# jgsimard/big-dreamer

Measured on AMD Instinct MI355X. Metric: latent transitions/sec (RSSM + imagination) at batch=50 chunk=50 H=15, higher is better.
Workload: dtype f32

## Files before the change

### big_dreamer_amd/csrc/bd_device.h

```cpp
#pragma once
#include <hip/hip_runtime.h>
#include <stdint.h>

namespace bd {

typedef float floatx4 __attribute__((ext_vector_type(4)));

#ifndef BD_WAVES
#define BD_WAVES 4
#endif
constexpr int kWaves = BD_WAVES;
constexpr int kThreads = kWaves * 64;
constexpr int kFragFloats = 256;

__device__ __forceinline__ floatx4 mfma16(float a, float b, floatx4 c) {
    return __builtin_amdgcn_mfma_f32_16x16x4f32(a, b, c, 0, 0, 0);
}

__host__ __device__ __forceinline__ int cdiv(int a, int b) { return (a + b - 1) / b; }

__device__ __forceinline__ int bd_tid() {
    int t = threadIdx.x;
    asm volatile("" : "+v"(t));
    return t;
}
static_assert((kWaves & (kWaves - 1)) == 0, "kWaves must be a power of two");
__device__ __forceinline__ int bd_wave(int tid) { return ((tid >> 6) + (int)blockIdx.x) & (kWaves - 1); }

#define BD_KARGS(T, name) const __attribute__((address_space(4))) T* name = \
    (const __attribute__((address_space(4))) T*)__builtin_amdgcn_kernarg_segment_ptr()
#define BD_KARGS_FRESH(name) asm volatile("" : "+s"(name))

__device__ __forceinline__ void lds_barrier() {
    asm volatile("s_waitcnt lgkmcnt(0)" ::: "memory");
    __builtin_amdgcn_s_barrier();
    asm volatile("" ::: "memory");
}

__device__ __forceinline__ int frag_idx(int row, int k) {
    return ((k >> 4) * 64 + ((k >> 2) & 3) * 16 + row) * 4 + (k & 3);
}

#ifdef BD_EXACT_MATH
__device__ __forceinline__ float elu(float x) { return x > 0.f ? x : expm1f(x); }
__device__ __forceinline__ float sigmoidf(float x) { return 1.f / (1.f + expf(-x)); }
__device__ __forceinline__ float tanh_act(float x) { return tanhf(x); }
__device__ __forceinline__ float softplusf(float x) { return x > 20.f ? x : log1pf(expf(x)); }
__device__ __forceinline__ float one_minus_exp_neg(float x) { return -expm1f(-x); }
#else
__device__ __forceinline__ float elu(float x) { return x > 0.f ? x : __expf(x) - 1.f; }
__device__ __forceinline__ float sigmoidf(float x) { return __builtin_amdgcn_rcpf(1.f + __expf(-x)); }
__device__ __forceinline__ float tanh_act(float x) { return 1.f - 2.f * __builtin_amdgcn_rcpf(__expf(2.f * x) + 1.f); }
__device__ __forceinline__ float softplusf(float x) { return x > 20.f ? x : __logf(1.f + __expf(x)); }
__device__ __forceinline__ float one_minus_exp_neg(float x) { return 1.f - __expf(-x); }
#endif
__device__ __forceinline__ float elu_grad_from_out(float y) { return y > 0.f ? 1.f : y + 1.f; }
__device__ __forceinline__ float act_apply(int act, float x) { return act ? elu(x) : x; }

__device__ __forceinline__ float wave_sum(float v) {
#pragma unroll
    for (int off = 32; off > 0; off >>= 1) v += __shfl_down(v, off, 64);
    return v;
}
__device__ __forceinline__ double wave_sum_d(double v) {
#pragma unroll
    for (int off = 32; off > 0; off >>= 1) v += __shfl_down(v, off, 64);
    return v;
}
__device__ __forceinline__ double block_sum_d(double v, double* red) {
    v = wave_sum_d(v);
    const int lane = threadIdx.x & 63, wave = threadIdx.x >> 6;
    __syncthreads();
    if (lane == 0) red[wave] = v;
    __syncthreads();
    double s = 0.0;
    if (bd_tid() == 0) {
        const int nw = (blockDim.x + 63) >> 6;
        for (int w = 0; w < nw; ++w) s += red[w];
    }
    return s;
}

template <int RT>
__device__ __forceinline__ void load_tile_concat(float* __restrict__ X, int Kb, int row0, int M,
                                                 const float* __restrict__ in0, int ld0, int w0,
                                                 const float* __restrict__ in1, int ld1, int w1,
                                                 float scale = 1.f) {
    const int Kp = Kb * 16;
    for (int idx = bd_tid(); idx < RT * 16 * Kp; idx += blockDim.x) {
        const int r = idx / Kp, k = idx - r * Kp;
        const int grow = row0 + r;
        float v = 0.f;
        if (grow < M) {
            if (k < w0) v = in0[(size_t)grow * ld0 + k];
            else if (k < w0 + w1) v = in1[(size_t)grow * ld1 + (k - w0)];
        }
        X[(r >> 4) * Kb * kFragFloats + frag_idx(r & 15, k)] = v * scale;
    }
}

__host__ __device__ __forceinline__ bool tile_pairs_ok(const float* in0, int ld0, int w0, const float* in1, int ld1) {
    return ((w0 | ld0) & 1) == 0 && ((uintptr_t)in0 & 7) == 0 && (in1 == nullptr || ((ld1 & 1) == 0 && ((uintptr_t)in1 & 7) == 0));
}
template <int RT>
__device__ __forceinline__ void load_tile_concat_pairs(float* __restrict__ X, int Kb, int row0, int M,
                                                       const float* __restrict__ in0, int ld0, int w0,
                                                       const float* __restrict__ in1, int ld1, int w1) {
    typedef float floatx2 __attribute__((ext_vector_type(2)));
    const int tid = bd_tid(), wave = tid >> 6, lane = tid & 63;
    const int Kp = Kb * 16, W = w0 + w1;
    constexpr int kRows = 16 * RT / kWaves;
    constexpr int kBatch = 6;
    static_assert(16 * RT % kWaves == 0, "rows must divide over the waves");
    for (int k = 2 * lane; k < Kp; k += 128) {
#pragma unroll
        for (int b0 = 0; b0 < kRows; b0 += kBatch) {
            floatx2 v[kBatch];
#pragma unroll
            for (int b = 0; b < kBatch; ++b) {
                const int r = wave + (b0 + b) * kWaves, grow = row0 + r;
                v[b] = floatx2{0.f, 0.f};
                if (b0 + b < kRows && grow < M) {
                    if (k < w0) v[b] = *reinterpret_cast<const floatx2*>(in0 + (size_t)grow * ld0 + k);
                    else if (k + 1 < W) v[b] = *reinterpret_cast<const floatx2*>(in1 + (size_t)grow * ld1 + (k - w0));
                    else if (k < W) v[b][0] = in1[(size_t)grow * ld1 + (k - w0)];
                }
            }
#pragma unroll
            for (int b = 0; b < kBatch; ++b) {
                const int r = wave + (b0 + b) * kWaves;
                if (b0 + b < kRows)
                    *reinterpret_cast<floatx2*>(X + (r >> 4) * Kb * kFragFloats + frag_idx(r & 15, k)) = v[b];
            }
        }
    }
}

template <int D, class LoadF, class MmaF>
__device__ __forceinline__ void pipelined_k(int Kb, LoadF&& load, MmaF&& mma) {
    using Frag = decltype(load(0));
    const int G = Kb / D, nt = Kb - G * D;
    Frag A[D], B[D];
    Frag T[D > 1 ? D - 1 : 1];
#pragma unroll
    for (int i = 0; i < D - 1; ++i)
        if (i < nt) T[i] = load(G * D + i);
    if (G > 0) {
#pragma unroll
        for (int i = 0; i < D; ++i) A[i] = load(i);
        int g = 1;
        for (; g + 1 < G; g += 2) {
#pragma unroll
            for (int i = 0; i < D; ++i) B[i] = load(g * D + i);
            __builtin_amdgcn_sched_barrier(0);
#pragma unroll
            for (int i = 0; i < D; ++i) mma(A[i]);
#pragma unroll
            for (int i = 0; i < D; ++i) A[i] = load((g + 1) * D + i);
            __builtin_amdgcn_sched_barrier(0);
#pragma unroll
            for (int i = 0; i < D; ++i) mma(B[i]);
        }
        if (g < G) {
#pragma unroll
            for (int i = 0; i < D; ++i) B[i] = load(g * D + i);
            __builtin_amdgcn_sched_barrier(0);
#pragma unroll
            for (int i = 0; i < D; ++i) mma(A[i]);
#pragma unroll
            for (int i = 0; i < D; ++i) mma(B[i]);
        } else {
#pragma unroll
// ... 486 lines not shown
            const size_t off = (size_t)nb * Kb * 64 + lane;
            const floatx4* __restrict__ W0 = reinterpret_cast<const floatx4*>(seg[s].W0) + off;
            const floatx4* __restrict__ W1 = reinterpret_cast<const floatx4*>(seg[s].W1) + off;
            if (seg[s].W0 != nullptr && seg[s].W1 != nullptr) {
                pipelined_k<2>(
                    Kb, [&](int kb) { return DualFrag{X4[kb * 64], W0[kb * 64], W1[kb * 64]}; },
                    [&](const DualFrag& f) {
#pragma unroll
                        for (int j = 0; j < 4; ++j) {
                            acc0 = mfma16(f.a[j], f.p[j], acc0);
                            acc1 = mfma16(f.a[j], f.q[j], acc1);
                        }
                    });
            } else if (seg[s].W0 != nullptr) {
                for (int kb = 0; kb < Kb; ++kb) {
                    const floatx4 a4 = X4[kb * 64], p4 = W0[kb * 64];
#pragma unroll
                    for (int j = 0; j < 4; ++j) acc0 = mfma16(a4[j], p4[j], acc0);
                }
            } else if (seg[s].W1 != nullptr) {
                for (int kb = 0; kb < Kb; ++kb) {
                    const floatx4 a4 = X4[kb * 64], q4 = W1[kb * 64];
#pragma unroll
                    for (int j = 0; j < 4; ++j) acc1 = mfma16(a4[j], q4[j], acc1);
                }
            }
        }
        epi(nb, acc0, acc1, pf);
    }
}

struct NoPre1 {
    __device__ __forceinline__ NoPreVal operator()(int) const { return NoPreVal{}; }
};
template <int NSEG, class Epi>
__device__ __forceinline__ void tile_linear_dual(const Seg2 (&seg)[NSEG], const float* __restrict__ bias0,
                                                 const float* __restrict__ bias1, int N, Epi&& epi,
                                                 float* __restrict__ scratch = nullptr) {
    tile_linear_dual_pre<NSEG>(seg, bias0, bias1, N, NoPre1{},
                               [&](int nb, floatx4 a0, floatx4 a1, NoPreVal) { epi(nb, a0, a1); }, scratch);
}

template <int NSEG, class PreE, class EpiE>
__device__ __forceinline__ void tile_dual_head_elem(const Seg2 (&seg)[NSEG], const float* __restrict__ bias0,
                                                    const float* __restrict__ bias1, int N, float* __restrict__ scratch,
                                                    PreE&& pre_elem, EpiE&& epi_elem, int sb = -1) {
    const int lane = bd_tid() & 63;
    const int Nb = (N + 15) >> 4, Np = Nb * 16;
    float* __restrict__ plain = scratch + kSplitPartialFloats;
    const int e0 = bd_tid();
    const int row0e = e0 / N, col0e = e0 - row0e * N;
    decltype(pre_elem(0, 0)) pv{};
    BD_DSTAMP(sb, 0);
#ifdef BD_STAMPS
    if (sb >= 0) asm volatile("s_waitcnt vmcnt(0)" ::: "memory");
    BD_DSTAMP(sb, 6);
#endif
    if (e0 < 16 * N) pv = pre_elem(row0e, col0e);
#ifdef BD_STAMPS
    if (sb >= 0) asm volatile("s_waitcnt vmcnt(0)" ::: "memory");
    BD_DSTAMP(sb, 7);
#endif
    BD_DSTAMP(sb, 1);
    tile_linear_dual_pre<NSEG>(
        seg, bias0, bias1, N, NoPre1{},
        [&](int nb, floatx4 a0, floatx4 a1, NoPreVal) {
#pragma unroll
            for (int r = 0; r < 4; ++r) {
                const int o = (4 * (lane >> 4) + r) * Np + nb * 16 + (lane & 15);
                plain[o] = a0[r];
                plain[16 * Np + o] = a1[r];
            }
        },
        Nb <= kSplitPairs ? scratch : nullptr, sb >= 0 ? sb + 16 : -1);
    BD_DSTAMP(sb, 2);
    lds_barrier();
    BD_DSTAMP(sb, 3);
#ifdef BD_STAMPS
    if (sb >= 0) asm volatile("s_waitcnt vmcnt(0)" ::: "memory");
    BD_DSTAMP(sb, 4);
#endif
    if (e0 < 16 * N) epi_elem(row0e, col0e, plain[row0e * Np + col0e], plain[16 * Np + row0e * Np + col0e], pv);
    BD_DSTAMP(sb, 5);
    for (int e = e0 + blockDim.x; e < 16 * N; e += blockDim.x) {
        const int row = e / N, col = e - row * N;
        epi_elem(row, col, plain[row * Np + col], plain[16 * Np + row * Np + col], pre_elem(row, col));
    }
}

#ifndef BD_GRU_PIPE3
#define BD_GRU_PIPE3 0
#endif
#if BD_GRU_PIPE3
#define BD_GRU_PIPE pipelined_k3
#else
#define BD_GRU_PIPE pipelined_k<1>
#endif

struct GruW {
    const float *w_ir, *w_iz, *w_in, *w_hr, *w_hz, *w_hn;
    const float *b_ih, *b_hh;
};

struct GruFrag {
    floatx4 ax, ah, bir, biz, bin, bhr, bhz, bhn;
};

struct GruHalfFrag {
    floatx4 ax, ah, b0, b1;
};

template <class Epi>
__device__ __forceinline__ void gru_block(const floatx4* __restrict__ X4, const floatx4* __restrict__ H4, int Kb, int Be,
                                          const GruW& w, int nb, int lane, Epi&& epi) {
    const int col = nb * 16 + (lane & 15);
    const bool ok = col < Be;
    const float br = ok ? w.b_ih[col] + w.b_hh[col] : 0.f;
    const float bz = ok ? w.b_ih[Be + col] + w.b_hh[Be + col] : 0.f;
    const float bni = ok ? w.b_ih[2 * Be + col] : 0.f;
    const float bnh = ok ? w.b_hh[2 * Be + col] : 0.f;
    floatx4 R = floatx4{br, br, br, br}, Z = floatx4{bz, bz, bz, bz};
    floatx4 NI = floatx4{bni, bni, bni, bni}, NH = floatx4{bnh, bnh, bnh, bnh};
    const size_t off = (size_t)nb * Kb * 64 + lane;
    const floatx4* __restrict__ Wir = reinterpret_cast<const floatx4*>(w.w_ir) + off;
    const floatx4* __restrict__ Wiz = reinterpret_cast<const floatx4*>(w.w_iz) + off;
    const floatx4* __restrict__ Win = reinterpret_cast<const floatx4*>(w.w_in) + off;
    const floatx4* __restrict__ Whr = reinterpret_cast<const floatx4*>(w.w_hr) + off;
    const floatx4* __restrict__ Whz = reinterpret_cast<const floatx4*>(w.w_hz) + off;
    const floatx4* __restrict__ Whn = reinterpret_cast<const floatx4*>(w.w_hn) + off;
    BD_GRU_PIPE(
        Kb,
        [&](int kb) {
            return GruFrag{X4[kb * 64], H4[kb * 64], Wir[kb * 64], Wiz[kb * 64], Win[kb * 64],
                           Whr[kb * 64], Whz[kb * 64], Whn[kb * 64]};
        },
        [&](const GruFrag& f) {
#pragma unroll
            for (int j = 0; j < 4; ++j) {
                R = mfma16(f.ax[j], f.bir[j], R);
                Z = mfma16(f.ax[j], f.biz[j], Z);
                NI = mfma16(f.ax[j], f.bin[j], NI);
                NH = mfma16(f.ah[j], f.bhn[j], NH);
                R = mfma16(f.ah[j], f.bhr[j], R);
                Z = mfma16(f.ah[j], f.bhz[j], Z);
            }
        });
    epi(nb, R, Z, NI, NH);
}

template <class Epi>
__device__ __forceinline__ void gru_tile(const float* __restrict__ X, const float* __restrict__ Hf, int Kb, int Be,
                                         const GruW& w, Epi&& epi, float* __restrict__ scratch = nullptr) {
    const int lane = bd_tid() & 63, wave = bd_wave(bd_tid());
    const int Nb = (Be + 15) >> 4;
    const floatx4* __restrict__ X4 = reinterpret_cast<const floatx4*>(X) + lane;
    const floatx4* __restrict__ H4 = reinterpret_cast<const floatx4*>(Hf) + lane;
    if (kWaves == 8 && Nb == 13 && scratch != nullptr) {
        gru_block(X4, H4, Kb, Be, w, wave, lane, epi);
        floatx4* __restrict__ S4 = reinterpret_cast<floatx4*>(scratch);
        if (wave < 4) {
            gru_block(X4, H4, Kb, Be, w, wave + 8, lane, epi);
        } else if (wave > 4) {
            const int nb = 12, col = nb * 16 + (lane & 15);
            const bool ok = col < Be;
            const int g = wave - 5;
            const float b0 = !ok ? 0.f : (g == 2 ? w.b_ih[2 * Be + col] : w.b_ih[g * Be + col] + w.b_hh[g * Be + col]);
            const float b1 = (ok && g == 2) ? w.b_hh[2 * Be + col] : 0.f;
            floatx4 A0 = floatx4{b0, b0, b0, b0}, A1 = floatx4{b1, b1, b1, b1};
            const size_t off = (size_t)nb * Kb * 64 + lane;
            const float* wx = g == 0 ? w.w_ir : (g == 1 ? w.w_iz : w.w_in);
            const float* wh = g == 0 ? w.w_hr : (g == 1 ? w.w_hz : w.w_hn);
            const floatx4* __restrict__ Wx = reinterpret_cast<const floatx4*>(wx) + off;
            const floatx4* __restrict__ Wh = reinterpret_cast<const floatx4*>(wh) + off;
            pipelined_k<2>(
                Kb, [&](int kb) { return GruHalfFrag{X4[kb * 64], H4[kb * 64], Wx[kb * 64], Wh[kb * 64]}; },
                [&](const GruHalfFrag& f) {
#pragma unroll
                    for (int j = 0; j < 4; ++j) {
                        A0 = mfma16(f.ax[j], f.b0[j], A0);
                        A1 = mfma16(f.ah[j], f.b1[j], A1);
                    }
                });
            if (g == 2) {
                S4[2 * 64 + lane] = A0;
                S4[3 * 64 + lane] = A1;
            } else {
                S4[g * 64 + lane] = A0 + A1;
            }
        }
        lds_barrier();
        if (wave == 4) epi(12, S4[lane], S4[64 + lane], S4[2 * 64 + lane], S4[3 * 64 + lane]);
        return;
    }
    for (int nb = wave; nb < Nb; nb += kWaves) gru_block(X4, H4, Kb, Be, w, nb, lane, epi);
}

struct GruWT {
    const float *wt_ir, *wt_iz, *wt_in, *wt_hr, *wt_hz, *wt_hn;
};

struct GruBwdFrag {
    floatx4 ar, az, ai, ah, bir, biz, bin, bhr, bhz, bhn;
};

template <class PF, class Epi>
__device__ __forceinline__ void gru_bwd_block(const floatx4* __restrict__ R4, const floatx4* __restrict__ Z4,
                                              const floatx4* __restrict__ I4, const floatx4* __restrict__ H4, int Kb,
                                              const GruWT& w, int nb, int lane, const PF& pf, Epi&& epi) {
    floatx4 DX = floatx4{0.f, 0.f, 0.f, 0.f}, DH = floatx4{0.f, 0.f, 0.f, 0.f};
    floatx4 DX2 = DX, DH2 = DH;
    const size_t off = (size_t)nb * Kb * 64 + lane;
    const floatx4* __restrict__ Wir = reinterpret_cast<const floatx4*>(w.wt_ir) + off;
    const floatx4* __restrict__ Wiz = reinterpret_cast<const floatx4*>(w.wt_iz) + off;
    const floatx4* __restrict__ Win = reinterpret_cast<const floatx4*>(w.wt_in) + off;
    const floatx4* __restrict__ Whr = reinterpret_cast<const floatx4*>(w.wt_hr) + off;
    const floatx4* __restrict__ Whz = reinterpret_cast<const floatx4*>(w.wt_hz) + off;
    const floatx4* __restrict__ Whn = reinterpret_cast<const floatx4*>(w.wt_hn) + off;
    BD_GRU_PIPE(
        Kb,
        [&](int kb) {
            return GruBwdFrag{R4[kb * 64], Z4[kb * 64], I4[kb * 64], H4[kb * 64], Wir[kb * 64], Wiz[kb * 64],
                              Win[kb * 64], Whr[kb * 64], Whz[kb * 64], Whn[kb * 64]};
        },
        [&](const GruBwdFrag& f) {
#pragma unroll
            for (int j = 0; j < 4; ++j) {
                DX = mfma16(f.ar[j], f.bir[j], DX);
                DH = mfma16(f.ar[j], f.bhr[j], DH);
                DX2 = mfma16(f.az[j], f.biz[j], DX2);
                DH2 = mfma16(f.az[j], f.bhz[j], DH2);
                DX = mfma16(f.ai[j], f.bin[j], DX);
                DH = mfma16(f.ah[j], f.bhn[j], DH);
            }
        });
    epi(nb, DX + DX2, DH + DH2, pf);
}

struct GruBwdHalfFrag {
    floatx4 ax, ah, bx, bh;
};

template <class Pre, class Epi>
__device__ __forceinline__ void gru_tile_bwd(const float* __restrict__ dR, const float* __restrict__ dZ,
                                             const float* __restrict__ dNI, const float* __restrict__ dNH, int Kb,
                                             int Be, const GruWT& w, Pre&& pre, Epi&& epi, float* __restrict__ scratch = nullptr) {
    const int lane = bd_tid() & 63, wave = bd_wave(bd_tid());
    const int Nb = (Be + 15) >> 4;
    const floatx4* __restrict__ R4 = reinterpret_cast<const floatx4*>(dR) + lane;
    const floatx4* __restrict__ Z4 = reinterpret_cast<const floatx4*>(dZ) + lane;
    const floatx4* __restrict__ I4 = reinterpret_cast<const floatx4*>(dNI) + lane;
    const floatx4* __restrict__ H4 = reinterpret_cast<const floatx4*>(dNH) + lane;
    if (kWaves == 8 && Nb == 13 && scratch != nullptr) {
        decltype(pre(0)) pf12{};
        if (wave == 4) pf12 = pre(12);
        gru_bwd_block(R4, Z4, I4, H4, Kb, w, wave, lane, pre(wave), epi);
        floatx4* __restrict__ S4 = reinterpret_cast<floatx4*>(scratch);
        if (wave < 4) {
            gru_bwd_block(R4, Z4, I4, H4, Kb, w, wave + 8, lane, pre(wave + 8), epi);
        } else if (wave > 4) {
            const int g = wave - 5;
            const size_t off = (size_t)12 * Kb * 64 + lane;
            const floatx4* __restrict__ Ax = g == 0 ? R4 : (g == 1 ? Z4 : I4);
            const floatx4* __restrict__ Ah = g == 0 ? R4 : (g == 1 ? Z4 : H4);
            const floatx4* __restrict__ Wx = reinterpret_cast<const floatx4*>(g == 0 ? w.wt_ir : (g == 1 ? w.wt_iz : w.wt_in)) + off;
            const floatx4* __restrict__ Wh = reinterpret_cast<const floatx4*>(g == 0 ? w.wt_hr : (g == 1 ? w.wt_hz : w.wt_hn)) + off;
            floatx4 DX = floatx4{0.f, 0.f, 0.f, 0.f}, DH = DX;
            pipelined_k<2>(
                Kb, [&](int kb) { return GruBwdHalfFrag{Ax[kb * 64], Ah[kb * 64], Wx[kb * 64], Wh[kb * 64]}; },
                [&](const GruBwdHalfFrag& f) {
#pragma unroll
                    for (int j = 0; j < 4; ++j) {
                        DX = mfma16(f.ax[j], f.bx[j], DX);
                        DH = mfma16(f.ah[j], f.bh[j], DH);
                    }
                });
            S4[(2 * g) * 64 + lane] = DX;
            S4[(2 * g + 1) * 64 + lane] = DH;
// ... 16 lines not shown
```

### big_dreamer_amd/csrc/imagine.hip

```cpp
#include "bd_device.h"
#include "bd_host.h"
#include "bd_scan.h"
#include "bd_rng.h"
#include "bd_discrete.h"

namespace bd {

constexpr int kMaxA = 64;

#ifdef BD_STAMPS
__device__ unsigned long long g_stamps[64];
#define BD_STAMP(slot)                                                                      \
    do {                                                                                    \
        if (blockIdx.x == BD_STAMP_WG && threadIdx.x == 0 && t == 3) g_stamps[slot] = __builtin_amdgcn_s_memtime(); \
    } while (0)
#ifndef BD_STAMP_WG
#define BD_STAMP_WG 0
#endif
#else
#define BD_STAMP(slot)
#endif

struct ImgDims {
    int Kb_h, Kb_s, Kb_a, Kb_hd;
    __host__ __device__ ImgDims(int Be, int S, int A, int Hd)
        : Kb_h(cdiv(Be, 16)), Kb_s(cdiv(S, 16)), Kb_a(cdiv(A, 16)), Kb_hd(cdiv(Hd, 16)) {}
};


__global__ __launch_bounds__(kThreads) void imagine_fwd_kernel(bd_imagine_fwd_args a_) {
    extern __shared__ __attribute__((aligned(16))) float smem[];
    BD_KARGS(bd_imagine_fwd_args, ap);
#define a (*ap)
    const ImgDims d(a.Be, a.S, a.A, a.Hd);
    const int row0 = blockIdx.x * 16;
    const int F = a.Be + a.S, A = a.A;
    const int nh = d.Kb_h * kFragFloats, nhd = d.Kb_hd * kFragFloats;
    float* h_cur = smem;
    float* h_nxt = h_cur + nh;
    float* xf = h_nxt + nh;
    float* bufA = xf + nh;
    float* bufB = bufA + nhd;
    float* sf = bufB + nhd;
    float* af = sf + d.Kb_s * kFragFloats;
    float* mean_s = af + d.Kb_a * kFragFloats;
    float* std_s = mean_s + 16 * A;
    float* lp_rj = std_s + 16 * A;
    float* part = lp_rj + 16 * A;
    float* scratch = part + kWaves * 16 * A * 3;

    load_tile_concat<1>(h_cur, d.Kb_h, row0, a.N, a.start_feat, F, a.Be, nullptr, 0, 0);
    load_tile_concat<1>(sf, d.Kb_s, row0, a.N, a.start_feat + a.Be, F, a.S, nullptr, 0, 0);
    for (int i = threadIdx.x; i < d.Kb_a * kFragFloats; i += blockDim.x) af[i] = 0.f;
    lds_barrier();

    const size_t act_stride = a.sv_actor_stride ? a.sv_actor_stride : (size_t)a.Hm * a.N * a.Hd;
    const float inv_ns = 1.f / (float)a.n_samples;

    for (int t = 0; t < a.Hm; ++t) {
        const size_t tn = (size_t)t * a.N;
        const int tid = bd_tid();
        const int lane = tid & 63, wave = bd_wave(tid);
        auto hidden_epi = [&](float* dst, float* save, size_t tn_, int width) {
            return HiddenEpiTR{dst, save, tn_, width, a.N, row0, lane};
        };
        BD_STAMP(0);
        BD_KARGS_FRESH(ap);
        {
            const Seg segs[2] = {{h_cur, a.w_a0h, d.Kb_h}, {sf, a.w_a0s, d.Kb_s}};
            tile_linear_seg_tr<2>(segs, a.b_a[0], a.Hd, hidden_epi(bufA, a.sv_actor, tn, a.Hd));
        }
        BD_STAMP(1);
        lds_barrier();
        BD_STAMP(2);
        BD_KARGS_FRESH(ap);
        {
            float* src = bufA;
            float* dst = bufB;
            for (int l = 1; l < 4; ++l) {
                const Seg segs[1] = {{src, a.w_a[l - 1], d.Kb_hd}};
                tile_linear_seg_tr<1>(segs, a.b_a[l], a.Hd,
                                      hidden_epi(dst, a.sv_actor ? a.sv_actor + l * act_stride : nullptr, tn, a.Hd),
                                      (t == 3 && l == 2) ? 32 : -1);
                BD_DSTAMP((t == 3 && l == 2) ? 32 : -1, 4);
                lds_barrier();
                BD_DSTAMP((t == 3 && l == 2) ? 32 : -1, 5);
                float* tmp = src; src = dst; dst = tmp;
            }
        }
        BD_STAMP(3);
        BD_KARGS_FRESH(ap);
        if (a.discrete_actions) {
            const Seg segs[1] = {{bufB, a.w_a4m, d.Kb_hd}};
            tile_linear_pre<1, 1>(segs, a.b_a4, A, NoPre{}, [&](int, int nb, floatx4 acc, NoPreVal) {
                const int col = nb * 16 + (lane & 15);
#pragma unroll
                for (int r = 0; r < 4; ++r)
                    if (col < A) mean_s[(4 * (lane >> 4) + r) * A + col] = acc[r];
            }, scratch);
            lds_barrier();
            disc_rows(mean_s, af, a.eps_action, a.action, a.entropy, a.sv_act_stats, tn, row0, a.N, A, lane, wave);
        } else {
            const Seg2 segs[1] = {{bufB, a.w_a4m, a.w_a4s, d.Kb_hd}};
            tile_dual_head_elem<1>(
                segs, a.b_a4, a.b_a4 + A, A, scratch,
                [&](int row, int col) { return row0 + row < a.N ? a.eps_action[(tn + row0 + row) * A + col] : 0.f; },
                [&](int row, int col, float Mn, float Rw, float eps) {
                    const int grow = row0 + row;
                    float act = 0.f;
                    if (grow < a.N) {
                        const float th = tanh_act(Mn / a.act_mean_scale);
                        const float mean = a.act_mean_scale * th;
                        const float pre = Rw + a.act_raw_init_std;
                        const float sd = softplusf(pre) + a.act_min_std;
                        const float u = mean + sd * eps;
                        act = tanh_act(u);
                        a.action[(tn + grow) * A + col] = act;
                        mean_s[row * A + col] = mean;
                        std_s[row * A + col] = sd;
                        if (a.sv_act_stats) {
                            float* st = a.sv_act_stats + (tn + grow) * 4 * A + col;
                            st[0] = th;
                            st[A] = sigmoidf(pre);
                            st[2 * A] = mean;
                            st[3 * A] = sd;
                        }
                        if (a.sv_act_us) {
                            float* us = a.sv_act_us + (tn + grow) * 2 * A + col;
                            us[0] = u;
                            us[A] = sd;
                        }
                    }
                    af[frag_idx(row, col)] = act;
                },
                t == 3 ? 0 : -1);
        }
        BD_STAMP(4);
        lds_barrier();
        BD_STAMP(5);
        BD_KARGS_FRESH(ap);
        if (a.sv_act_stats == nullptr && !a.discrete_actions) {
            const int row = tid & 15, sl = tid >> 4;
            const int grow = row0 + row;
            for (int j = 0; j < A; ++j) {
                float lp = 0.f, dm = 0.f, ds = 0.f;
                if (grow < a.N) {
                    const EntConst ec = entropy_const(mean_s[row * A + j], std_s[row * A + j]);
                    for (int k = sl; k < a.n_samples; k += kThreads / 16) {
                        const float e = a.eps_entropy[(((size_t)t * a.n_samples + k) * a.N + grow) * A + j];
                        float l1, d1, d2;
                        entropy_sample(ec, e, l1, d1, d2);
                        lp += l1; dm += d1; ds += d2;
                    }
                }
                lp += __shfl_xor(lp, 16, 64); lp += __shfl_xor(lp, 32, 64);
                dm += __shfl_xor(dm, 16, 64); dm += __shfl_xor(dm, 32, 64);
                ds += __shfl_xor(ds, 16, 64); ds += __shfl_xor(ds, 32, 64);
                if (lane < 16) {
                    float* p = part + ((wave * 16 + row) * A + j) * 3;
                    p[0] = lp; p[1] = dm; p[2] = ds;
                }
            }
            lds_barrier();
            for (int i = tid; i < 16 * A; i += blockDim.x) {
                const int row = i / A, j = i - row * A;
                float lp = 0.f;
                for (int w = 0; w < kWaves; ++w) lp += part[((w * 16 + row) * A + j) * 3];
                lp_rj[i] = lp;
            }
            lds_barrier();
            if (tid < 16 && row0 + tid < a.N) {
                float s = 0.f;
                for (int j = 0; j < A; ++j) s += lp_rj[tid * A + j];
                a.entropy[tn + row0 + tid] = -s * inv_ns;
            }
        }
        BD_STAMP(6);
        BD_KARGS_FRESH(ap);
        {
            const Seg segs[2] = {{sf, a.w_embed_s, d.Kb_s}, {af, a.w_embed_a, d.Kb_a}};
            tile_linear_seg_tr<2>(segs, a.b_embed, a.Be, hidden_epi(xf, a.sv_x, tn, a.Be));
        }
        BD_STAMP(7);
        lds_barrier();
        BD_STAMP(8);
        BD_KARGS_FRESH(ap);
        const GruW gw{a.w_ir, a.w_iz, a.w_in, a.w_hr, a.w_hz, a.w_hn, a.b_ih, a.b_hh};
        gru_tile(xf, h_cur, d.Kb_h, a.Be, gw, [&](int nb, floatx4 R, floatx4 Z, floatx4 NI, floatx4 NH) {
            const int c = lane & 15, q = lane >> 4;
            const int off0 = acc_frag_off(nb, lane, 0);
            if (row0 + 16 <= a.N && nb * 16 + 16 <= a.Be) {
                float rr[4], zz[4], nn[4], hn[4];
#pragma unroll
                for (int r = 0; r < 4; ++r) {
                    rr[r] = sigmoidf(R[r]);
                    zz[r] = sigmoidf(Z[r]);
                    nn[r] = tanh_act(NI[r] + rr[r] * NH[r]);
                    hn[r] = (1.f - zz[r]) * nn[r] + zz[r] * h_cur[off0 + 4 * r];
                }
#pragma unroll
                for (int r = 0; r < 4; ++r) h_nxt[off0 + 4 * r] = hn[r];
                const unsigned lo = (unsigned)(row0 + 4 * q), cc = (unsigned)(nb * 16 + c);
                float* __restrict__ f = a.feat + tn * F + (lo * (unsigned)F + cc);
#pragma unroll
                for (int r = 0; r < 4; ++r) st_save(f + (unsigned)r * (unsigned)F, hn[r]);
                if (a.sv_gates) {
                    const unsigned Be = (unsigned)a.Be;
                    float* __restrict__ g = a.sv_gates + tn * 4 * a.Be + (lo * 4u * Be + cc);
#pragma unroll
                    for (int r = 0; r < 4; ++r) {
                        float* gr = g + (unsigned)r * 4u * Be;
                        st_save(gr, rr[r]); st_save(gr + Be, zz[r]); st_save(gr + 2u * Be, nn[r]); st_save(gr + 3u * Be, NH[r]);
                    }
                }
                return;
            }
            const int col = nb * 16 + c;
#pragma unroll
            for (int r = 0; r < 4; ++r) {
                const int grow = row0 + 4 * q + r;
                const int off = off0 + 4 * r;
                const float rr = sigmoidf(R[r]), zz = sigmoidf(Z[r]);
                const float nn = tanh_act(NI[r] + rr * NH[r]);
                const float hn = (1.f - zz) * nn + zz * h_cur[off];
                const bool ok = grow < a.N && col < a.Be;
                h_nxt[off] = ok ? hn : 0.f;
                if (ok) {
                    a.feat[(tn + grow) * F + col] = hn;
                    if (a.sv_gates) {
                        float* g = a.sv_gates + (tn + grow) * 4 * a.Be + col;
                        g[0] = rr; g[a.Be] = zz; g[2 * a.Be] = nn; g[3 * a.Be] = NH[r];
                    }
                }
            }
        }, scratch);
        BD_STAMP(9);
        lds_barrier();
        BD_STAMP(10);
        BD_KARGS_FRESH(ap);
        {
            const Seg segs[1] = {{h_nxt, a.w_p1, d.Kb_h}};
            tile_linear_seg_tr<1>(segs, a.b_p1, a.Hd, hidden_epi(bufA, a.sv_p, tn, a.Hd));
        }
        BD_STAMP(11);
        lds_barrier();
        BD_STAMP(12);
        BD_KARGS_FRESH(ap);
        {
            const Seg2 segs[1] = {{bufA, a.w_p2m, a.w_p2s, d.Kb_hd}};
            tile_dual_head_elem<1>(
                segs, a.b_p2, a.b_p2 + a.S, a.S, scratch,
                [&](int row, int col) { return row0 + row < a.N ? a.eps_prior[(tn + row0 + row) * a.S + col] : 0.f; },
                [&](int row, int col, float Mn, float Rw, float eps) {
                    const int grow = row0 + row;
                    float st = 0.f;
                    if (grow < a.N) {
                        const size_t i = (tn + grow) * a.S + col;
                        const float sd = softplusf(Rw) + a.min_std;
                        st = Mn + sd * eps;
                        if (a.prior_mean) a.prior_mean[i] = Mn;
                        a.prior_std[i] = sd;
                        a.feat[(tn + grow) * F + a.Be + col] = st;
                    }
                    sf[frag_idx(row, col)] = st;
                },
                t == 3 ? 8 : -1);
        }
        BD_STAMP(13);
        lds_barrier();
        BD_STAMP(14);
        float* tmp = h_cur; h_cur = h_nxt; h_nxt = tmp;
    }
#undef a
}

constexpr int kEntParts = 16;
template <bool RNG>
__global__ __launch_bounds__(64 * kEntParts) void actor_entropy_kernel(const float* __restrict__ eps, float* __restrict__ stats,
                                                            float* __restrict__ entropy, int Hm, int N, int A, int ns, Rng rng) {
    __shared__ float red[kEntParts][64][3];
    __shared__ float lpj[64];
    const int lane = threadIdx.x & 63, part = threadIdx.x >> 6;
    const int rows_pb = 64 / A;
    const int rl = lane / A, j = lane - rl * A;
    const long row = (long)blockIdx.x * rows_pb + rl;
    const bool valid = rl < rows_pb && row < (long)Hm * N;
    float lp = 0.f, dm = 0.f, ds = 0.f;
    if (valid) {
        const int t = (int)(row / N), n = (int)(row - (long)t * N);
        const float* st = stats + (size_t)row * 4 * A + j;
        const EntConst ec = entropy_const(st[2 * A], st[3 * A]);
        if constexpr (RNG) {
            const int mine = (ns - part + kEntParts - 1) / kEntParts;
            const uint64_t base = (((uint64_t)row * A + j) * kEntParts + part) * (uint64_t)((ns / kEntParts + 4) / 4);
            for (int k0 = 0; k0 < mine; k0 += 4) {
                float e[4];
                rng_normal4(rng, base + (k0 >> 2), e);
#pragma unroll
                for (int q = 0; q < 4; ++q)
                    if (k0 + q < mine) {
                        float l1, d1, d2;
                        entropy_sample(ec, e[q], l1, d1, d2);
                        lp += l1; dm += d1; ds += d2;
                    }
            }
        } else {
            const float* e0 = eps + ((size_t)t * ns * N + n) * A + j;
            for (int k = part; k < ns; k += kEntParts) {
                float l1, d1, d2;
                entropy_sample(ec, e0[(size_t)k * N * A], l1, d1, d2);
                lp += l1; dm += d1; ds += d2;
            }
        }
    }
    red[part][lane][0] = lp; red[part][lane][1] = dm; red[part][lane][2] = ds;
    __syncthreads();
    const float inv_ns = 1.f / (float)ns;
    if (part == 0) {
        float a0 = 0.f, a1 = 0.f, a2 = 0.f;
        for (int w = 0; w < kEntParts; ++w) { a0 += red[w][lane][0]; a1 += red[w][lane][1]; a2 += red[w][lane][2]; }
        lpj[lane] = a0;
        if (valid) {
            float* st = stats + (size_t)row * 4 * A + j;
            st[2 * A] = -a1 * inv_ns;
            st[3 * A] = -a2 * inv_ns;
        }
    }
    __syncthreads();
    if (part == 0 && valid && j == 0) {
        float s = 0.f;
        for (int jj = 0; jj < A; ++jj) s += lpj[lane + jj];
        entropy[row] = -s * inv_ns;
// ... 184 lines not shown
                    }
                    return p;
                },
                [&](int, int nb, floatx4 acc, const PreAct& p) {
                    const int col = nb * 16 + (lane & 15);
#pragma unroll
                    for (int r = 0; r < 4; ++r) {
                        const int grow = row0 + 4 * (lane >> 4) + r;
                        float gm = 0.f, gr = 0.f;
                        if (grow < a.N && col < A) {
                            const float dxa = acc[r] * (1.f - p.act[r] * p.act[r]);
                            const float dent = a.ent_weight ? a.dentropy * a.ent_weight[tn + grow] : a.dentropy;
                            const float dmean = dxa + dent * p.dm[r];
                            const float dstd = dxa * p.eps[r] + dent * p.ds[r];
                            gm = dmean * (1.f - p.th[r] * p.th[r]);
                            gr = dstd * p.sg[r];
                            a.d_actor_out[(tn + grow) * 2 * A + col] = gm;
                            a.d_actor_out[(tn + grow) * 2 * A + A + col] = gr;
                        }
                        dAm[acc_frag_off(nb, lane, r)] = gm;
                        dAr[acc_frag_off(nb, lane, r)] = gr;
                    }
                },
                scratch);
        }
        lds_barrier();
        BD_KARGS_FRESH(ap);
        BD_STAMP(25);
        if (a.d_actor_pre != nullptr) {
        {
            const Seg segs[2] = {{dAm, a.wt_a4m, d.Kb_a}, {dAr, a.wt_a4s, d.Kb_a}};
            tile_linear_pre<1, 2>(segs, nullptr, a.Hd, dpre_pre(a.sv_actor + 3 * act_stride, tn, a.Hd),
                                  dpre_epi(bufA, a.d_actor_pre + 3 * act_stride, tn, a.Hd));
        }
        lds_barrier();
        {
            float* src = bufA;
            float* dst = bufB;
            for (int l = 2; l >= 0; --l) {
                const Seg segs[1] = {{src, a.wt_a[l], d.Kb_hd}};
                tile_linear_pre<1, 1>(segs, nullptr, a.Hd, dpre_pre(a.sv_actor + l * act_stride, tn, a.Hd),
                                      dpre_epi(l > 0 ? dst : nullptr, a.d_actor_pre + l * act_stride, tn, a.Hd));
                lds_barrier();
                float* tmp = src; src = dst; dst = tmp;
            }
        }
        }
        BD_STAMP(26);
    }
#undef a
}

}

extern "C" {
using namespace bd;

#ifdef BD_STAMPS
int bd_debug_stamps(unsigned long long* out64) {
    return hipMemcpyFromSymbol(out64, HIP_SYMBOL(g_stamps), sizeof(unsigned long long) * 64) == hipSuccess ? 0 : -1;
}
int bd_debug_dstamps(unsigned long long* out64) {
    return hipMemcpyFromSymbol(out64, HIP_SYMBOL(g_dstamps), sizeof(unsigned long long) * 64) == hipSuccess ? 0 : -1;
}
#endif

static int imagine_forward_scan(const bd_imagine_fwd_args* a, void* stream) {
    BD_REQUIRE(a && a->N > 0 && a->Hm > 0 && a->Be > 0 && a->S > 0 && a->A > 0 && a->A <= kMaxA && a->Hd > 0 &&
                   a->n_samples > 0, "bd_imagine_forward: bad dims");
    BD_REQUIRE(a->S <= kHeadMaxN && a->A <= kHeadMaxN, "bd_imagine_forward: state / action width above %d", kHeadMaxN);
    BD_REQUIRE(a->w_embed_s && a->w_embed_a && a->b_embed && a->w_ir && a->w_iz && a->w_in && a->w_hr && a->w_hz &&
                   a->w_hn && a->b_ih && a->b_hh && a->w_p1 && a->b_p1 && a->w_p2m && a->w_p2s && a->b_p2,
               "bd_imagine_forward: missing world-model weights");
    BD_REQUIRE(a->w_a0h && a->w_a0s && a->w_a[0] && a->w_a[1] && a->w_a[2] && a->b_a[0] && a->b_a[1] && a->b_a[2] &&
                   a->b_a[3] && a->w_a4m && (a->w_a4s || a->discrete_actions) && a->b_a4,
               "bd_imagine_forward: missing actor weights");
    BD_REQUIRE(!a->discrete_actions || a->sv_act_us == nullptr,
               "bd_imagine_forward: sv_act_us is for the tanh-Normal actor only (discrete_actions = 1 saves norm in sv_act_stats)");
    BD_REQUIRE(a->start_feat && a->eps_action && a->eps_prior && (a->eps_entropy || a->sv_act_stats || a->discrete_actions),
               "bd_imagine_forward: missing inputs (eps_entropy may be NULL only with sv_act_stats: the entropy estimate is then "
               "the caller's bd_actor_entropy / bd_actor_entropy_rng launch)");
    BD_REQUIRE(a->feat && a->prior_std && a->entropy && a->action, "bd_imagine_forward: missing outputs");
    const ImgDims d(a->Be, a->S, a->A, a->Hd);
    const size_t lds = ((size_t)(3 * d.Kb_h + 2 * d.Kb_hd + d.Kb_s + d.Kb_a) * kFragFloats +
                        (size_t)(3 * 16 + kWaves * 16 * 3) * a->A + kSplitScratchFloats) * sizeof(float);
    BD_REQUIRE(lds <= (size_t)kMaxLds, "bd_imagine_forward: needs %zu B of LDS", lds);
    if (lds > 64 * 1024 && allow_big_lds(imagine_fwd_kernel)) return -1;
    hipLaunchKernelGGL(imagine_fwd_kernel, dim3(cdiv(a->N, 16)), dim3(kThreads), lds, (hipStream_t)stream, *a);
    BD_CHECK_LAUNCH("bd_imagine_forward");
    return 0;
}

int bd_actor_entropy(const float* eps_entropy, float* act_stats, float* entropy, int Hm, int N, int A, int n_samples,
                     void* stream) {
    BD_REQUIRE(eps_entropy && act_stats && entropy && Hm > 0 && N > 0 && A > 0 && A <= kMaxA && n_samples > 0,
               "bd_actor_entropy: bad arguments");
    const int rows_pb = 64 / A;
    hipLaunchKernelGGL(actor_entropy_kernel<false>, dim3(cdiv(Hm * N, rows_pb)), dim3(64 * kEntParts), 0, (hipStream_t)stream,
                       eps_entropy, act_stats, entropy, Hm, N, A, n_samples, Rng{0, 0, 0, 0});
    BD_CHECK_LAUNCH("bd_actor_entropy");
    return 0;
}

int bd_actor_entropy_rng(unsigned long long seed, unsigned long long step, unsigned stream_id, float* act_stats, float* entropy,
                         int Hm, int N, int A, int n_samples, void* stream) {
    BD_REQUIRE(act_stats && entropy && Hm > 0 && N > 0 && A > 0 && A <= kMaxA && n_samples > 0, "bd_actor_entropy_rng: bad arguments");
    const int rows_pb = 64 / A;
    hipLaunchKernelGGL(actor_entropy_kernel<true>, dim3(cdiv(Hm * N, rows_pb)), dim3(64 * kEntParts), 0, (hipStream_t)stream,
                       nullptr, act_stats, entropy, Hm, N, A, n_samples,
                       Rng{(uint32_t)seed, (uint32_t)(seed >> 32), stream_id, (uint32_t)step});
    BD_CHECK_LAUNCH("bd_actor_entropy_rng");
    return 0;
}

int bd_imagine_forward_scan(const bd_imagine_fwd_args* a, void* stream) { return imagine_forward_scan(a, stream); }

int bd_imagine_forward(const bd_imagine_fwd_args* a, void* stream) {
    if (int rc = imagine_forward_scan(a, stream)) return rc;
    if (a->sv_act_stats != nullptr && a->eps_entropy != nullptr && !a->discrete_actions)
        return bd_actor_entropy(a->eps_entropy, a->sv_act_stats, a->entropy, a->Hm, a->N, a->A, a->n_samples, stream);
    return 0;
}

int bd_imagine_backward(const bd_imagine_bwd_args* a, void* stream) {
    BD_REQUIRE(a && a->N > 0 && a->Hm > 0 && a->Be > 0 && a->S > 0 && a->A > 0 && a->A <= kMaxA && a->Hd > 0,
               "bd_imagine_backward: bad dims");
    BD_REQUIRE(a->wt_embed_s && a->wt_embed_a && a->wt_ir && a->wt_iz && a->wt_in && a->wt_hr && a->wt_hz && a->wt_hn &&
                   a->wt_p1 && a->wt_p2m && a->wt_p2s && a->wt_a[0] && a->wt_a[1] && a->wt_a[2] &&
                   (a->discrete_actions || (a->wt_a4m && a->wt_a4s)),
               "bd_imagine_backward: missing weights");
    BD_REQUIRE(!a->discrete_actions || a->d_actor_pre == nullptr,
               "bd_imagine_backward: the Categorical actor's hidden layers run as the caller's chain (d_actor_pre = NULL)");
    BD_REQUIRE(a->start_feat && a->feat && a->prior_std && a->action && (a->eps_action || a->discrete_actions) &&
                   a->eps_prior && a->sv_actor &&
                   a->sv_act_stats && a->sv_x && a->sv_gates && a->sv_p && a->dfeat,
               "bd_imagine_backward: missing forward tensors");
    BD_REQUIRE(a->d_actor_out, "bd_imagine_backward: missing outputs");
    const ImgDims d(a->Be, a->S, a->A, a->Hd);
    const size_t lds = ((size_t)(6 * d.Kb_h + 3 * d.Kb_hd + 2 * d.Kb_s + 2 * d.Kb_a) * kFragFloats + 16 * a->S +
                        kSplitPartialFloats) * sizeof(float);
    BD_REQUIRE(lds <= (size_t)kMaxLds, "bd_imagine_backward: needs %zu B of LDS", lds);
    if (lds > 64 * 1024 && allow_big_lds(imagine_bwd_kernel)) return -1;
    hipLaunchKernelGGL(imagine_bwd_kernel, dim3(cdiv(a->N, 16)), dim3(kThreads), lds, (hipStream_t)stream, *a);
    BD_CHECK_LAUNCH("bd_imagine_backward");
    return 0;
}

}
```

Measured before the change: 13.33 million.

## Pack two row tiles per imagine block and add lean GRU gate path

The imagine forward kernel now runs two independent 16-row tiles per workgroup, each wave group using its own compacted LDS region (buffers are aliased to shrink per-tile footprint), with a waves-per-EU hint. A leaner GRU block splits the r/z and n gate accumulations into two passes to cut live registers and prefetch depth. The aim is higher occupancy and fewer blocks. The risk is the extra LDS per block and the doubled X/H fragment loads in the lean GRU path.

New measurement: 11.26 million. 0.845x the previous value.

```diff
diff --git a/big_dreamer_amd/csrc/bd_device.h b/big_dreamer_amd/csrc/bd_device.h
--- a/big_dreamer_amd/csrc/bd_device.h
+++ b/big_dreamer_amd/csrc/bd_device.h
@@ -19,13 +19,25 @@
 
 __host__ __device__ __forceinline__ int cdiv(int a, int b) { return (a + b - 1) / b; }
 
+#ifdef BD_TILE_GROUPS
+__device__ __forceinline__ int bd_group() { return __builtin_amdgcn_readfirstlane((int)threadIdx.x / (kWaves * 64)); }
+__device__ __forceinline__ int bd_tile() { return (int)blockIdx.x * ((int)blockDim.x / (kWaves * 64)) + bd_group(); }
+__device__ __forceinline__ int bd_group_threads() { return kWaves * 64; }
+#else
+__device__ __forceinline__ int bd_tile() { return (int)blockIdx.x; }
+__device__ __forceinline__ int bd_group_threads() { return (int)blockDim.x; }
+#endif
 __device__ __forceinline__ int bd_tid() {
+#ifdef BD_TILE_GROUPS
+    int t = threadIdx.x & (kWaves * 64 - 1);
+#else
     int t = threadIdx.x;
+#endif
     asm volatile("" : "+v"(t));
     return t;
 }
 static_assert((kWaves & (kWaves - 1)) == 0, "kWaves must be a power of two");
-__device__ __forceinline__ int bd_wave(int tid) { return ((tid >> 6) + (int)blockIdx.x) & (kWaves - 1); }
+__device__ __forceinline__ int bd_wave(int tid) { return ((tid >> 6) + bd_tile()) & (kWaves - 1); }
 
 #define BD_KARGS(T, name) const __attribute__((address_space(4))) T* name = \
     (const __attribute__((address_space(4))) T*)__builtin_amdgcn_kernarg_segment_ptr()
@@ -87,7 +99,7 @@
                                                  const float* __restrict__ in1, int ld1, int w1,
                                                  float scale = 1.f) {
     const int Kp = Kb * 16;
-    for (int idx = bd_tid(); idx < RT * 16 * Kp; idx += blockDim.x) {
+    for (int idx = bd_tid(); idx < RT * 16 * Kp; idx += bd_group_threads()) {
         const int r = idx / Kp, k = idx - r * Kp;
         const int grow = row0 + r;
         float v = 0.f;
@@ -740,7 +752,7 @@
 #endif
     if (e0 < 16 * N) epi_elem(row0e, col0e, plain[row0e * Np + col0e], plain[16 * Np + row0e * Np + col0e], pv);
     BD_DSTAMP(sb, 5);
-    for (int e = e0 + blockDim.x; e < 16 * N; e += blockDim.x) {
+    for (int e = e0 + bd_group_threads(); e < 16 * N; e += bd_group_threads()) {
         const int row = e / N, col = e - row * N;
         epi_elem(row, col, plain[row * Np + col], plain[16 * Np + row * Np + col], pre_elem(row, col));
     }
@@ -806,7 +818,56 @@
     epi(nb, R, Z, NI, NH);
 }
 
+struct GruGateFrag {
+    floatx4 ax, ah, bxr, bxz, bhr, bhz;
+};
 template <class Epi>
+__device__ __forceinline__ void gru_block_lean(const floatx4* __restrict__ X4, const floatx4* __restrict__ H4, int Kb, int Be,
+                                               const GruW& w, int nb, int lane, Epi&& epi) {
+    const int col = nb * 16 + (lane & 15);
+    const bool ok = col < Be;
+    const size_t off = (size_t)nb * Kb * 64 + lane;
+    floatx4 R, Z;
+    {
+        const float br = ok ? w.b_ih[col] + w.b_hh[col] : 0.f;
+        const float bz = ok ? w.b_ih[Be + col] + w.b_hh[Be + col] : 0.f;
+        R = floatx4{br, br, br, br};
+        Z = floatx4{bz, bz, bz, bz};
+        const floatx4* __restrict__ Wir = reinterpret_cast<const floatx4*>(w.w_ir) + off;
+        const floatx4* __restrict__ Wiz = reinterpret_cast<const floatx4*>(w.w_iz) + off;
+        const floatx4* __restrict__ Whr = reinterpret_cast<const floatx4*>(w.w_hr) + off;
+        const floatx4* __restrict__ Whz = reinterpret_cast<const floatx4*>(w.w_hz) + off;
+        pipelined_k<1>(
+            Kb,
+            [&](int kb) { return GruGateFrag{X4[kb * 64], H4[kb * 64], Wir[kb * 64], Wiz[kb * 64], Whr[kb * 64], Whz[kb * 64]}; },
+            [&](const GruGateFrag& f) {
+#pragma unroll
+                for (int j = 0; j < 4; ++j) {
+                    R = mfma16(f.ax[j], f.bxr[j], R);
+                    Z = mfma16(f.ax[j], f.bxz[j], Z);
+                    R = mfma16(f.ah[j], f.bhr[j], R);
+                    Z = mfma16(f.ah[j], f.bhz[j], Z);
+                }
+            });
+    }
+    const float bni = ok ? w.b_ih[2 * Be + col] : 0.f;
+    const float bnh = ok ? w.b_hh[2 * Be + col] : 0.f;
+    floatx4 NI = floatx4{bni, bni, bni, bni}, NH = floatx4{bnh, bnh, bnh, bnh};
+    const floatx4* __restrict__ Win = reinterpret_cast<const floatx4*>(w.w_in) + off;
+    const floatx4* __restrict__ Whn = reinterpret_cast<const floatx4*>(w.w_hn) + off;
+    pipelined_k<1>(
+        Kb, [&](int kb) { return GruHalfFrag{X4[kb * 64], H4[kb * 64], Win[kb * 64], Whn[kb * 64]}; },
+        [&](const GruHalfFrag& f) {
+#pragma unroll
+            for (int j = 0; j < 4; ++j) {
+                NI = mfma16(f.ax[j], f.b0[j], NI);
+                NH = mfma16(f.ah[j], f.b1[j], NH);
+            }
+        });
+    epi(nb, R, Z, NI, NH);
+}
+
+template <bool LEAN = false, class Epi>
 __device__ __forceinline__ void gru_tile(const float* __restrict__ X, const float* __restrict__ Hf, int Kb, int Be,
                                          const GruW& w, Epi&& epi, float* __restrict__ scratch = nullptr) {
     const int lane = bd_tid() & 63, wave = bd_wave(bd_tid());
@@ -814,10 +875,14 @@
     const floatx4* __restrict__ X4 = reinterpret_cast<const floatx4*>(X) + lane;
     const floatx4* __restrict__ H4 = reinterpret_cast<const floatx4*>(Hf) + lane;
     if (kWaves == 8 && Nb == 13 && scratch != nullptr) {
-        gru_block(X4, H4, Kb, Be, w, wave, lane, epi);
+        auto block = [&](int nb) {
+            if constexpr (LEAN) gru_block_lean(X4, H4, Kb, Be, w, nb, lane, epi);
+            else gru_block(X4, H4, Kb, Be, w, nb, lane, epi);
+        };
+        block(wave);
         floatx4* __restrict__ S4 = reinterpret_cast<floatx4*>(scratch);
         if (wave < 4) {
-            gru_block(X4, H4, Kb, Be, w, wave + 8, lane, epi);
+            block(wave + 8);
         } else if (wave > 4) {
             const int nb = 12, col = nb * 16 + (lane & 15);
             const bool ok = col < Be;
@@ -830,7 +895,7 @@
             const float* wh = g == 0 ? w.w_hr : (g == 1 ? w.w_hz : w.w_hn);
             const floatx4* __restrict__ Wx = reinterpret_cast<const floatx4*>(wx) + off;
             const floatx4* __restrict__ Wh = reinterpret_cast<const floatx4*>(wh) + off;
-            pipelined_k<2>(
+            pipelined_k<LEAN ? 1 : 2>(
                 Kb, [&](int kb) { return GruHalfFrag{X4[kb * 64], H4[kb * 64], Wx[kb * 64], Wh[kb * 64]}; },
                 [&](const GruHalfFrag& f) {
 #pragma unroll
@@ -850,7 +915,15 @@
         if (wave == 4) epi(12, S4[lane], S4[64 + lane], S4[2 * 64 + lane], S4[3 * 64 + lane]);
         return;
     }
-    for (int nb = wave; nb < Nb; nb += kWaves) gru_block(X4, H4, Kb, Be, w, nb, lane, epi);
+    for (int nb = wave; nb < Nb; nb += kWaves) {
+        if constexpr (LEAN) {
+            int nbo = nb;
+            asm volatile("" : "+v"(nbo));
+            gru_block_lean(X4, H4, Kb, Be, w, nbo, lane, epi);
+        } else {
+            gru_block(X4, H4, Kb, Be, w, nb, lane, epi);
+        }
+    }
 }
 
 struct GruWT {
diff --git a/big_dreamer_amd/csrc/imagine.hip b/big_dreamer_amd/csrc/imagine.hip
--- a/big_dreamer_amd/csrc/imagine.hip
+++ b/big_dreamer_amd/csrc/imagine.hip
@@ -1,3 +1,4 @@
+#define BD_TILE_GROUPS
 #include "bd_device.h"
 #include "bd_host.h"
 #include "bd_scan.h"
@@ -28,41 +29,59 @@
 };
 
 
-__global__ __launch_bounds__(kThreads) void imagine_fwd_kernel(bd_imagine_fwd_args a_) {
+struct ImgFwdLds {
+    int h1, bx, sf, af, mean, std, work, total;
+    __host__ __device__ ImgFwdLds(const ImgDims& d, int A) {
+        const int nh = d.Kb_h * kFragFloats, nhd = d.Kb_hd * kFragFloats;
+        const int head = kSplitPartialFloats + 2 * 16 * 16 * (d.Kb_s > d.Kb_a ? d.Kb_s : d.Kb_a);
+        const int ent = (kWaves * 3 + 1) * 16 * A;
+        int w = nhd > head ? nhd : head;
+        w = w > ent ? w : ent;
+        h1 = nh;
+        bx = h1 + nh;
+        sf = bx + (nh > nhd ? nh : nhd);
+        af = sf + d.Kb_s * kFragFloats;
+        mean = af + d.Kb_a * kFragFloats;
+        std = mean + 16 * A;
+        work = std + 16 * A;
+        total = work + w;
+    }
+};
+
+constexpr int kImgFwdTiles = 2;
+__global__ __launch_bounds__(kImgFwdTiles * kThreads) __attribute__((amdgpu_waves_per_eu(4, 4)))
+void imagine_fwd_kernel(bd_imagine_fwd_args a_) {
     extern __shared__ __attribute__((aligned(16))) float smem[];
     BD_KARGS(bd_imagine_fwd_args, ap);
 #define a (*ap)
     const ImgDims d(a.Be, a.S, a.A, a.Hd);
-    const int row0 = blockIdx.x * 16;
+    const int row0 = bd_tile() * 16;
     const int F = a.Be + a.S, A = a.A;
-    const int nh = d.Kb_h * kFragFloats, nhd = d.Kb_hd * kFragFloats;
-    float* h_cur = smem;
-    float* h_nxt = h_cur + nh;
-    float* xf = h_nxt + nh;
-    float* bufA = xf + nh;
-    float* bufB = bufA + nhd;
-    float* sf = bufB + nhd;
-    float* af = sf + d.Kb_s * kFragFloats;
-    float* mean_s = af + d.Kb_a * kFragFloats;
-    float* std_s = mean_s + 16 * A;
-    float* lp_rj = std_s + 16 * A;
-    float* part = lp_rj + 16 * A;
-    float* scratch = part + kWaves * 16 * A * 3;
+    const ImgFwdLds L(d, A);
+    float* h_cur = smem + __builtin_amdgcn_readfirstlane(bd_group() * L.total);
+    float* h_nxt = h_cur + L.h1;
+    float* bufB = h_cur + L.bx;
+    float* xf = bufB;
+    float* sf = h_cur + L.sf;
+    float* af = h_cur + L.af;
+    float* mean_s = h_cur + L.mean;
+    float* std_s = h_cur + L.std;
+    float* bufA = h_cur + L.work;
+    float* scratch = bufA;
+    float* part = bufA;
+    float* lp_rj = part + kWaves * 16 * A * 3;
 
     load_tile_concat<1>(h_cur, d.Kb_h, row0, a.N, a.start_feat, F, a.Be, nullptr, 0, 0);
     load_tile_concat<1>(sf, d.Kb_s, row0, a.N, a.start_feat + a.Be, F, a.S, nullptr, 0, 0);
-    for (int i = threadIdx.x; i < d.Kb_a * kFragFloats; i += blockDim.x) af[i] = 0.f;
+    for (int i = bd_tid(); i < d.Kb_a * kFragFloats; i += kThreads) af[i] = 0.f;
     lds_barrier();
 
     const size_t act_stride = a.sv_actor_stride ? a.sv_actor_stride : (size_t)a.Hm * a.N * a.Hd;
-    const float inv_ns = 1.f / (float)a.n_samples;
 
     for (int t = 0; t < a.Hm; ++t) {
         const size_t tn = (size_t)t * a.N;
-        const int tid = bd_tid();
-        const int lane = tid & 63, wave = bd_wave(tid);
         auto hidden_epi = [&](float* dst, float* save, size_t tn_, int width) {
-            return HiddenEpiTR{dst, save, tn_, width, a.N, row0, lane};
+            return HiddenEpiTR{dst, save, tn_, width, a.N, row0, bd_tid() & 63};
         };
         BD_STAMP(0);
         BD_KARGS_FRESH(ap);
@@ -91,6 +110,7 @@
         BD_STAMP(3);
         BD_KARGS_FRESH(ap);
         if (a.discrete_actions) {
+            const int lane = bd_tid() & 63, wave = bd_wave(bd_tid());
             const Seg segs[1] = {{bufB, a.w_a4m, d.Kb_hd}};
             tile_linear_pre<1, 1>(segs, a.b_a4, A, NoPre{}, [&](int, int nb, floatx4 acc, NoPreVal) {
                 const int col = nb * 16 + (lane & 15);
@@ -140,6 +160,7 @@
         BD_STAMP(5);
         BD_KARGS_FRESH(ap);
         if (a.sv_act_stats == nullptr && !a.discrete_actions) {
+            const int tid = bd_tid(), lane = tid & 63, wave = bd_wave(tid);
             const int row = tid & 15, sl = tid >> 4;
             const int grow = row0 + row;
             for (int j = 0; j < A; ++j) {
@@ -162,7 +183,7 @@
                 }
             }
             lds_barrier();
-            for (int i = tid; i < 16 * A; i += blockDim.x) {
+            for (int i = tid; i < 16 * A; i += kThreads) {
                 const int row = i / A, j = i - row * A;
                 float lp = 0.f;
                 for (int w = 0; w < kWaves; ++w) lp += part[((w * 16 + row) * A + j) * 3];
@@ -172,7 +193,7 @@
             if (tid < 16 && row0 + tid < a.N) {
                 float s = 0.f;
                 for (int j = 0; j < A; ++j) s += lp_rj[tid * A + j];
-                a.entropy[tn + row0 + tid] = -s * inv_ns;
+                a.entropy[tn + row0 + tid] = -s * (1.f / (float)a.n_samples);
             }
         }
         BD_STAMP(6);
@@ -186,7 +207,8 @@
         BD_STAMP(8);
         BD_KARGS_FRESH(ap);
         const GruW gw{a.w_ir, a.w_iz, a.w_in, a.w_hr, a.w_hz, a.w_hn, a.b_ih, a.b_hh};
-        gru_tile(xf, h_cur, d.Kb_h, a.Be, gw, [&](int nb, floatx4 R, floatx4 Z, floatx4 NI, floatx4 NH) {
+        gru_tile<true>(xf, h_cur, d.Kb_h, a.Be, gw, [&](int nb, floatx4 R, floatx4 Z, floatx4 NI, floatx4 NH) {
+            const int lane = bd_tid() & 63;
             const int c = lane & 15, q = lane >> 4;
             const int off0 = acc_frag_off(nb, lane, 0);
             if (row0 + 16 <= a.N && nb * 16 + 16 <= a.Be) {
@@ -216,6 +238,8 @@
                 return;
             }
             const int col = nb * 16 + c;
+            float* f0 = a.feat + (tn + row0 + 4 * q) * F + col;
+            float* g0 = a.sv_gates ? a.sv_gates + (tn + row0 + 4 * q) * 4 * a.Be + col : nullptr;
 #pragma unroll
             for (int r = 0; r < 4; ++r) {
                 const int grow = row0 + 4 * q + r;
@@ -226,9 +250,9 @@
                 const bool ok = grow < a.N && col < a.Be;
                 h_nxt[off] = ok ? hn : 0.f;
                 if (ok) {
-                    a.feat[(tn + grow) * F + col] = hn;
-                    if (a.sv_gates) {
-                        float* g = a.sv_gates + (tn + grow) * 4 * a.Be + col;
+                    f0[r * F] = hn;
+                    if (g0) {
+                        float* g = g0 + r * 4 * a.Be;
                         g[0] = rr; g[a.Be] = zz; g[2 * a.Be] = nn; g[3 * a.Be] = NH[r];
                     }
                 }
@@ -240,14 +264,14 @@
         BD_KARGS_FRESH(ap);
         {
             const Seg segs[1] = {{h_nxt, a.w_p1, d.Kb_h}};
-            tile_linear_seg_tr<1>(segs, a.b_p1, a.Hd, hidden_epi(bufA, a.sv_p, tn, a.Hd));
+            tile_linear_seg_tr<1>(segs, a.b_p1, a.Hd, hidden_epi(bufB, a.sv_p, tn, a.Hd));
         }
         BD_STAMP(11);
         lds_barrier();
         BD_STAMP(12);
         BD_KARGS_FRESH(ap);
         {
-            const Seg2 segs[1] = {{bufA, a.w_p2m, a.w_p2s, d.Kb_hd}};
+            const Seg2 segs[1] = {{bufB, a.w_p2m, a.w_p2s, d.Kb_hd}};
             tile_dual_head_elem<1>(
                 segs, a.b_p2, a.b_p2 + a.S, a.S, scratch,
                 [&](int row, int col) { return row0 + row < a.N ? a.eps_prior[(tn + row0 + row) * a.S + col] : 0.f; },
@@ -598,11 +622,11 @@
                "the caller's bd_actor_entropy / bd_actor_entropy_rng launch)");
     BD_REQUIRE(a->feat && a->prior_std && a->entropy && a->action, "bd_imagine_forward: missing outputs");
     const ImgDims d(a->Be, a->S, a->A, a->Hd);
-    const size_t lds = ((size_t)(3 * d.Kb_h + 2 * d.Kb_hd + d.Kb_s + d.Kb_a) * kFragFloats +
-                        (size_t)(3 * 16 + kWaves * 16 * 3) * a->A + kSplitScratchFloats) * sizeof(float);
+    const size_t lds = (size_t)kImgFwdTiles * ImgFwdLds(d, a->A).total * sizeof(float);
     BD_REQUIRE(lds <= (size_t)kMaxLds, "bd_imagine_forward: needs %zu B of LDS", lds);
     if (lds > 64 * 1024 && allow_big_lds(imagine_fwd_kernel)) return -1;
-    hipLaunchKernelGGL(imagine_fwd_kernel, dim3(cdiv(a->N, 16)), dim3(kThreads), lds, (hipStream_t)stream, *a);
+    hipLaunchKernelGGL(imagine_fwd_kernel, dim3(cdiv(a->N, 16 * kImgFwdTiles)), dim3(kImgFwdTiles * kThreads), lds,
+                       (hipStream_t)stream, *a);
     BD_CHECK_LAUNCH("bd_imagine_forward");
     return 0;
 }
```
